# youtalk/opencv-ar

Hardware: AMD Instinct MI355X
Metric: frames/sec at 1920x1080, 16 markers/frame; 1/2/4/8 MI355X (higher is better)
Workload: dtype u8

## Files before the change

include/ocvar_hip.h:

```cpp
#ifndef OCVAR_HIP_H
#define OCVAR_HIP_H

#include <stddef.h>
#include <stdint.h>

#ifdef __cplusplus
extern "C" {
#endif

typedef struct { int width, height; double cameraMatrix[9]; double distCoeffs[5]; double glProjection[16]; } OcvarCamera;
typedef struct { int width, height; double scale; long long code[4]; } OcvarTemplate;
typedef struct {
    double glMatrix[16]; int templateId; int markerId; double score; float square[8]; double aspectRatio;
} OcvarMarker;

typedef struct {
    int markerId, templateId, orient, valid;
    long long bit;
    float square[8];
    float patPoint[8];
} OcvarCandidate;

typedef struct OcvarHip OcvarHip;

// ... 195 lines not shown
int ocvar_hip_debug_binary(OcvarHip* ctx, int frame, uint8_t* h_bin );
int ocvar_hip_debug_masks(OcvarHip* ctx, int frame, uint8_t* h_masks );
int ocvar_hip_debug_frame_quads(OcvarHip* ctx, int frame, int* quads , int* n_quads);
int ocvar_hip_debug_candidates(OcvarHip* ctx, int frame, OcvarCandidate* cands, int max_cands, int* n_cands);
typedef struct OcvarCropRoi {
    int index, frame, owner, x0, y0, w, h;
} OcvarCropRoi;
int ocvar_hip_debug_crop_rois(OcvarHip* ctx, OcvarCropRoi* rois, int max_rois, int* n_rois);
int ocvar_hip_debug_crop_plane(OcvarHip* ctx, int roi, int masks, uint8_t* h_plane );

typedef struct OcvarStart {
    int roi, x, y, is_hole;
} OcvarStart;
int ocvar_hip_debug_starts(OcvarHip* ctx, int crop_pass, OcvarStart* starts, int max_starts, int* n_starts);

int ocvar_hip_debug_calibrate(OcvarHip* ctx, size_t bytes);

int ocvar_hip_stage_ms(OcvarHip* ctx, float* ms, int n);
int ocvar_hip_stage_stamps(OcvarHip* ctx, void* ref_event, float* ms, int n);
int ocvar_hip_counters(OcvarHip* ctx, long long* out, int n);

#ifdef __cplusplus
}
#endif
#endif
```

opencv-ar_amd/__init__.py:

```python
import ctypes as C
import os

import numpy as np

_HERE = os.path.dirname(os.path.abspath(__file__))
LIB_DIR = os.path.join(_HERE, "lib")
HIP_LIB = os.environ.get("OCVAR_HIP_LIB") or os.path.join(LIB_DIR, "libocvar_hip.so")
SYNTH_LIB = os.path.join(LIB_DIR, "libocvar_synth.so")
HOST_LIB = os.path.join(LIB_DIR, "libopencv-ar.so.1.0.0")

MAX_TEMPLATES, MAX_TEMPLATE_SIZES, MAX_QUADS, MAX_MARKERS = 4096, 16, 256, 64
MAX_QUADS_EX, MAX_QUADS_DENSE, MAX_MARKERS_DENSE = 1792, 16384, 4096

HIP_SYMBOLS = [
    "ocvar_hip_create", "ocvar_hip_create_ex", "ocvar_hip_create_dense", "ocvar_hip_max_markers", "ocvar_hip_capacity_flags", "ocvar_hip_gate_create", "ocvar_hip_gate_create_lanes", "ocvar_hip_gate_lanes", "ocvar_hip_gate_destroy", "ocvar_hip_set_gate", "ocvar_hip_ready", "ocvar_hip_set_result_limit",
    "ocvar_hip_pipe_create", "ocvar_hip_pipe_destroy", "ocvar_hip_pipe_last_error", "ocvar_hip_pipe_set_templates", "ocvar_hip_pipe_set_camera",
    "ocvar_hip_pipe_detect_device", "ocvar_hip_pipe_track_device", "ocvar_hip_pipe_submit", "ocvar_hip_pipe_collect", "ocvar_hip_pipe_in_flight", "ocvar_hip_pipe_set_result_limit", "ocvar_hip_set_input_format", "ocvar_hip_pipe_set_input_format", "ocvar_hip_set_corner_refine", "ocvar_hip_pipe_set_corner_refine", "ocvar_hip_enqueue_tracked", "ocvar_hip_build_info", "ocvar_hip_set_tuning", "ocvar_hip_destroy", "ocvar_hip_last_error", "ocvar_hip_set_templates", "ocvar_hip_set_camera",
    "ocvar_hip_detect_device", "ocvar_hip_enqueue", "ocvar_hip_collect", "ocvar_hip_detect_host", "ocvar_hip_find_squares",
    "ocvar_hip_debug_gray", "ocvar_hip_debug_binary", "ocvar_hip_debug_masks", "ocvar_hip_debug_frame_quads", "ocvar_hip_debug_candidates",
    "ocvar_hip_debug_crop_rois", "ocvar_hip_debug_crop_plane", "ocvar_hip_debug_starts",
    "ocvar_hip_stage_ms", "ocvar_hip_stream", "ocvar_hip_stage_stamps", "ocvar_hip_counters", "ocvar_hip_results_to_device", "ocvar_hip_results_to_device_ex", "ocvar_hip_debug_calibrate",
    "ocvar_hip_set_board", "ocvar_hip_board_poses", "ocvar_hip_board_poses_to_device",
    "ocvar_hip_set_overlay", "ocvar_hip_render", "ocvar_hip_render_records",
    "ocvar_hip_annotate_default_style", "ocvar_hip_annotate", "ocvar_hip_annotate_records",
    "ocvar_hip_patches", "ocvar_hip_patches_records",
    "ocvar_hip_undistort", "ocvar_hip_undistort_records",
    "ocvar_hip_flow_records",
    "ocvar_hip_yuv_to_frames", "ocvar_hip_frames_to_yuv",
    "ocvar_hip_resize", "ocvar_hip_scale_records",
    "ocvar_hip_orient", "ocvar_hip_orient_records", "ocvar_hip_orient_camera",
    "ocvar_hip_warp", "ocvar_hip_warp_records", "ocvar_hip_board_plane_maps",
    "ocvar_hip_levels_default_params", "ocvar_hip_levels",
]
INPUT_FORMATS = {"bgr": 0, "rgb": 1, "bgra": 2, "rgba": 3, "gray": 4}
FORMAT_BPP = {0: 3, 1: 3, 2: 4, 3: 4, 4: 1}
# ... 314 lines not shown
        lib.ocvar_hip_set_templates.argtypes = [vp, vp, i]
        lib.ocvar_hip_set_camera.argtypes = [vp, vp]
        lib.ocvar_hip_detect_device.argtypes = [vp, vp, i, i, i, sz, i, i, vp, vp, vp, vp, i]
        lib.ocvar_hip_enqueue.argtypes = [vp, vp, i, i, i, sz, i, i, vp, vp, vp]
        lib.ocvar_hip_collect.argtypes = [vp, vp, vp, i]
        lib.ocvar_hip_detect_host.argtypes = [vp, vp, i, i, i, sz, i, i, vp, vp, vp, vp, i]
        lib.ocvar_hip_find_squares.argtypes = [vp, vp, i, i, i, vp, i, vp]
        lib.ocvar_hip_debug_gray.argtypes = [vp, i, vp]
        lib.ocvar_hip_debug_binary.argtypes = [vp, i, vp]
        lib.ocvar_hip_debug_masks.argtypes = [vp, i, vp]
        lib.ocvar_hip_debug_frame_quads.argtypes = [vp, i, vp, vp]
        lib.ocvar_hip_debug_candidates.argtypes = [vp, i, vp, i, vp]
        lib.ocvar_hip_debug_crop_rois.argtypes = [vp, vp, i, vp]
        lib.ocvar_hip_debug_crop_plane.argtypes = [vp, i, i, vp]
        lib.ocvar_hip_debug_starts.argtypes = [vp, i, vp, i, vp]
        lib.ocvar_hip_stage_ms.argtypes = [vp, vp, i]
        lib.ocvar_hip_counters.argtypes = [vp, vp, i]
        lib.ocvar_hip_stage_stamps.argtypes = [vp, vp, vp, i]
        lib.ocvar_hip_stream.argtypes = [vp]
        lib.ocvar_hip_stream.restype = vp
        lib.ocvar_hip_results_to_device.argtypes = [vp, vp, vp, vp]
        lib.ocvar_hip_results_to_device_ex.argtypes = [vp, vp, vp, i, vp]
        lib.ocvar_hip_debug_calibrate.argtypes = [vp, sz]
        lib.ocvar_hip_set_board.argtypes = [vp, vp, i]
        lib.ocvar_hip_board_poses.argtypes = [vp, vp, i]
        lib.ocvar_hip_board_poses_to_device.argtypes = [vp, vp, vp]
        lib.ocvar_hip_set_overlay.argtypes = [vp, i, vp, i, i, i]
        lib.ocvar_hip_render.argtypes = [vp, vp, i, i, i, sz, i, vp]
        lib.ocvar_hip_render_records.argtypes = [vp, vp, i, i, i, sz, i, i, vp, vp, i, vp]
        lib.ocvar_hip_annotate_default_style.argtypes = [vp]
# ... 589 lines not shown
        return out

    def debug_crop_binary(self, roi):
        return self._debug_crop_plane(roi, False)

    def debug_crop_masks(self, roi):
        return self._debug_crop_plane(roi, True)

    def debug_starts(self, crop_pass=False):
        n = C.c_int(0)
        self._check(self._lib.ocvar_hip_debug_starts(self._ctx, int(bool(crop_pass)), None, 0, C.byref(n)), "debug_starts")
        out = np.zeros(max(n.value, 1), START_DTYPE)
        self._check(self._lib.ocvar_hip_debug_starts(self._ctx, int(bool(crop_pass)), _ptr(out), n.value, C.byref(n)), "debug_starts")
        return out[:n.value]

    def stage_ms(self):
        ms = np.zeros(12, np.float32)
        k = self._lib.ocvar_hip_stage_ms(self._ctx, _ptr(ms), 12)
        return ms[:max(k, 0)]

    def stream_ptr(self):
        return self._lib.ocvar_hip_stream(self._ctx)

    def stage_stamps(self, ref_event):
        ms = np.zeros(13, np.float32)
        k = self._lib.ocvar_hip_stage_stamps(self._ctx, ref_event, _ptr(ms), 13)
        return ms[:max(k, 0)]

    def counters(self, n=10):
        out = np.zeros(n, np.int64)
# ... 3 lines not shown
```

opencv-ar_amd/csrc/api.hip:

```cpp
#include "context.h"
#include "plan_core.h"
#include <algorithm>
#include <cstdlib>
#include <cstring>
#include <new>

using namespace ocvar;

static_assert(sizeof(TemplateRec) == sizeof(OcvarTemplate) && sizeof(TemplateRec) == 48, "CvarTemplate layout");
static_assert(MAX_SIZE_CLASSES == OCVAR_MAX_TEMPLATE_SIZES, "size classes");
static_assert(sizeof(CameraRec) == sizeof(OcvarCamera) && sizeof(CameraRec) == 248, "CvarCamera layout");
static_assert(sizeof(MarkerRec) == sizeof(OcvarMarker) && sizeof(MarkerRec) == 184, "CvarMarker layout");
static_assert(sizeof(BoardEntry) == sizeof(OcvarBoardMarker) && sizeof(BoardEntry) == 72, "OcvarBoardMarker layout");
static_assert(sizeof(BoardPose) == sizeof(OcvarBoardPose) && sizeof(BoardPose) == 192, "OcvarBoardPose layout");

template <typename T>
static int dev_alloc(OcvarHip* c, T** p, size_t n) {
    void* q = nullptr;
    HIP_TRY(c, hipMalloc(&q, n * sizeof(T) + 256));
    c->allocs.push_back(q);
    *p = static_cast<T*>(q);
    return OCVAR_OK;
}

// ... 39 lines not shown
    if ((rc = dev_alloc(c, &w.crop_live, (size_t)w.cap_long))) return rc;
    if ((rc = dev_alloc(c, &w.long_frame, (size_t)w.cap_long))) return rc;
    if ((rc = dev_alloc(c, &w.long_crop, (size_t)w.cap_long))) return rc;
    if ((rc = dev_alloc(c, &w.quads_frame, B * max_quads))) return rc;
    if ((rc = dev_alloc(c, &w.n_quads_frame, B))) return rc;
    if ((rc = dev_alloc(c, &w.squares, B * max_quads * 8))) return rc;
    if ((rc = dev_alloc(c, &w.n_squares, B))) return rc;
    if ((rc = dev_alloc(c, &w.crop_of, B * max_quads))) return rc;
    if ((rc = dev_alloc(c, &w.rois_crop, (size_t)w.cap_crop_rois))) return rc;
    if ((rc = dev_alloc(c, &w.tiles_crop, (size_t)w.cap_crop_tiles))) return rc;
    if ((rc = dev_alloc(c, &w.quads_crop, (size_t)w.cap_crop_quads))) return rc;
    if ((rc = dev_alloc(c, &w.best_crop, (size_t)w.cap_crop_rois))) return rc;
    if ((rc = dev_alloc(c, &w.crop_min_rest, (size_t)w.cap_crop_rois))) return rc;
    if ((rc = dev_alloc(c, &w.ring_frame, B))) return rc;
    if ((rc = dev_alloc(c, &w.ring_crop, (size_t)w.cap_crop_rois))) return rc;
    if ((rc = dev_alloc(c, &w.sq_recs, B * max_quads))) return rc;
    if ((rc = dev_alloc(c, &w.prev, B * M))) return rc;
    if ((rc = dev_alloc(c, &w.n_prev, B))) return rc;
    if ((rc = dev_alloc(c, &w.reserve, B * M))) return rc;
    if ((rc = dev_alloc(c, &w.n_reserve, B))) return rc;
    if ((rc = dev_alloc(c, &w.markers, B * M))) return rc;
    if ((rc = dev_alloc(c, &w.pose_jobs, B * M))) return rc;
    if (dense) {
        const int nc = w.track_gw * w.track_gh;
        if ((rc = dev_alloc(c, &w.sorted_starts, B * max_quads))) return rc;
        if ((rc = dev_alloc(c, &w.sq_tmp, B * max_quads * 8))) return rc;
        if ((rc = dev_alloc(c, &w.trk_cells, B * (nc + 1)))) return rc;
        if ((rc = dev_alloc(c, &w.trk_fill, B * nc))) return rc;
        if ((rc = dev_alloc(c, &w.trk_items, B * 4 * max_quads))) return rc;
        if ((rc = dev_alloc(c, &w.trk_next, B * (max_quads + 1)))) return rc;
        if ((rc = dev_alloc(c, &w.surv, B * max_quads))) return rc;
        if ((rc = dev_alloc(c, &w.src, B * M))) return rc;
    }
    if ((rc = dev_alloc(c, &w.n_markers, B))) return rc;
    if ((rc = dev_alloc(c, &w.templates, (size_t)MAXT))) return rc;
    if ((rc = dev_alloc(c, &w.sizes, (size_t)MAX_SIZE_CLASSES))) return rc;
    if ((rc = dev_alloc(c, &w.lut, (size_t)4 * MAXT))) return rc;
    if ((rc = dev_alloc(c, &w.group_off, (size_t)MAXT + 1))) return rc;
    if ((rc = dev_alloc(c, &w.group_members, (size_t)MAXT))) return rc;
    if ((rc = dev_alloc(c, &w.camera, (size_t)1))) return rc;
    if ((rc = dev_alloc(c, &w.counters, (size_t)CNT_COUNT))) return rc;

    w.crop_pixels = reinterpret_cast<unsigned long long*>(w.counters + CNT_CROP_PIXELS);
    HIP_TRY(c, hipMemset(w.n_prev, 0, B * sizeof(int)));
    HIP_TRY(c, hipMemset(w.counters, 0, CNT_COUNT * sizeof(int)));
    HIP_TRY(c, c->h_markers.reserve(B * M * sizeof(MarkerRec)));
    HIP_TRY(c, c->h_counts.reserve(B * sizeof(int)));
    HIP_TRY(c, c->h_prev.reserve(B * M * sizeof(MarkerRec)));
    HIP_TRY(c, c->h_prev_counts.reserve(B * sizeof(int)));
    HIP_TRY(c, c->h_counters.reserve(CNT_COUNT * sizeof(int)));
    return OCVAR_OK;
}

extern "C" int ocvar_hip_create(OcvarHip** out, int device, int max_width, int max_height, int max_batch) {
    return ocvar_hip_create_ex(out, device, max_width, max_height, max_batch, OCVAR_MAX_QUADS);
}

extern "C" int ocvar_hip_create_ex(OcvarHip** out, int device, int max_width, int max_height, int max_batch, int max_quads) {
    if (max_quads < 1 || max_quads > OCVAR_MAX_QUADS_EX) return OCVAR_E_ARG;
    return create_impl(out, device, max_width, max_height, max_batch, max_quads, OCVAR_MAX_MARKERS, false);
// ... 157 lines not shown
        return OCVAR_E_ARG;
    }
    HIP_TRY(c, hipSetDevice(c->device));
    c->batch_board = false;
    c->crops_ran = false;
    plan_batch(&w, r.width, r.height, n_frames, c->gate != nullptr,
               PlanOverrides{tuned(c, OCVAR_TUNE_CROP_PHASES, "OCVAR_CROP_PHASES"), tuned(c, OCVAR_TUNE_MID_STEPS, "OCVAR_MID_STEPS"),
                             tuned(c, OCVAR_TUNE_MID_BLOCKS, "OCVAR_MID_BLOCKS"), tuned(c, OCVAR_TUNE_LONG_BLOCKS, "OCVAR_LONG_BLOCKS"),
                             tuned(c, OCVAR_TUNE_SHORT_BLOCKS, "OCVAR_SHORT_BLOCKS"), tuned(c, OCVAR_TUNE_MIN_UNITS, "OCVAR_MIN_UNITS")});
    if (after && after != s && hipStreamQuery(after) != hipSuccess) {
        (void)hipGetLastError();
        HIP_TRY(c, c->ordered.ensure(hipEventDisableTiming));
        HIP_TRY(c, hipEventRecord(c->ordered, after));
        HIP_TRY(c, hipStreamWaitEvent(s, c->ordered, 0));
    }
    HIP_TRY(c, hipMemsetAsync(w.counters, 0, CNT_COUNT * sizeof(int), s));
    HIP_TRY(c, hipMemsetAsync(w.n_quads_frame, 0, n_frames * sizeof(int), s));
    if (r.prev && r.prev_counts && r.prev_on_device) {
        HIP_TRY(c, hipMemcpyAsync(w.prev, r.prev, (size_t)n_frames * w.maxm * sizeof(MarkerRec), hipMemcpyDeviceToDevice, s));
        HIP_TRY(c, hipMemcpyAsync(w.n_prev, r.prev_counts, n_frames * sizeof(int), hipMemcpyDeviceToDevice, s));
    } else if (r.prev && r.prev_counts) {
        std::memcpy(c->h_prev, r.prev, (size_t)n_frames * w.maxm * sizeof(MarkerRec));
        std::memcpy(c->h_prev_counts, r.prev_counts, n_frames * sizeof(int));
        HIP_TRY(c, hipMemcpyAsync(w.prev, c->h_prev, (size_t)n_frames * w.maxm * sizeof(MarkerRec), hipMemcpyHostToDevice, s));
        HIP_TRY(c, hipMemcpyAsync(w.n_prev, c->h_prev_counts, n_frames * sizeof(int), hipMemcpyHostToDevice, s));
    } else {
        HIP_TRY(c, hipMemsetAsync(w.n_prev, 0, n_frames * sizeof(int), s));
    }
    const int hp_mask = (int)knob_or(tuned(c, OCVAR_TUNE_HP_MASK, "OCVAR_HP_MASK"), HP_MASK_DEFAULT) & 0x1ff;
    if (hp_mask && !c->hp_stream) {
        int lo = 0, hi = 0;
// ... 1105 lines not shown
```

opencv-ar_amd/csrc/binarise.hip:

```cpp
#include "kernels.h"
#include "starts_core.h"
#include <cstdlib>
#include <type_traits>

#ifndef OCVAR_WAVES_F
#define OCVAR_WAVES_F 5
#endif
#ifndef OCVAR_ROWS_AHEAD_F
#define OCVAR_ROWS_AHEAD_F 2
#endif
#ifndef OCVAR_ROWS_AHEAD_F4
#define OCVAR_ROWS_AHEAD_F4 1
#endif
#ifndef OCVAR_BIN_WG_WAVES
#define OCVAR_BIN_WG_WAVES 1
#endif
#ifndef OCVAR_ROWS_AHEAD_C
#define OCVAR_ROWS_AHEAD_C 1
#endif
#ifndef OCVAR_WAVES_C
#define OCVAR_WAVES_C 5
#endif

namespace ocvar {
// ... 50 lines not shown
    if constexpr (B == 1) asm("v_cmp_lt_i32_sdwa vcc, sext(%1), %2 src0_sel:WORD_1 src1_sel:BYTE_1\n\tv_cndmask_b32_e64 %0, 0, 1, vcc" : "=v"(nib) : "v"(S), "v"(w) : "vcc");
    if constexpr (B == 2) asm("v_cmp_lt_i32_sdwa vcc, sext(%1), %2 src0_sel:WORD_1 src1_sel:BYTE_2\n\tv_cndmask_b32_e64 %0, 0, 1, vcc" : "=v"(nib) : "v"(S), "v"(w) : "vcc");
    if constexpr (B == 3) asm("v_cmp_lt_i32_sdwa vcc, sext(%1), %2 src0_sel:WORD_1 src1_sel:BYTE_3\n\tv_cndmask_b32_e64 %0, 0, 1, vcc" : "=v"(nib) : "v"(S), "v"(w) : "vcc");
}

struct MarchOut {
    uint8_t* gray;
    long long gray_stride;
    uint8_t* nbr;
    int ns;
    int roi;
    StartCand* cands;
    int* n_cands;
    int cap_cands;
    int* err;
};

constexpr int SRC_CROP = 5;
constexpr int src_bpp(int src) { return src == OCVAR_FMT_BGR || src == OCVAR_FMT_RGB ? 3 : src == OCVAR_FMT_BGRA || src == OCVAR_FMT_RGBA ? 4 : 1; }

template <int SRC, bool EDGE>
__device__ void march_unit(const uint8_t* src, long long src_stride, int x_org , int sw, int sh, int strip, int Y0, int Y1, const MarchOut& o,
                           unsigned* stage, uint8_t* rowbuf ) {
    constexpr bool FRAME = SRC != SRC_CROP;
    constexpr int BPP = src_bpp(SRC);
    constexpr bool FOUR = BPP == 4;
    const int lane = threadIdx.x & 63;
    const int XS = strip * SV - 4 * HL;
    const int c0 = XS + 4 * lane;
    const int pw = sw >> 1, ph_ = sh >> 1;
// ... 41 lines not shown
            const unsigned e = stage[i];
            if (base + i < o.cap_cands) {
                StartCand sc;
                sc.roi = o.roi;
                sc.pos = (int)(e & 0x7fffffffu);
                sc.is_hole = (int)(e >> 31);
                o.cands[base + i] = sc;
            } else {
                atomicOr(o.err, ERR_CAND_OVERFLOW);
            }
        }
        __builtin_amdgcn_fence(__ATOMIC_ACQ_REL, "workgroup");
        staged = 0;
    };

    const int tile_s = strip * (SV / NBR_TILE_W) + (lane >> 2);
    const unsigned flush_src = (unsigned)(lane < 60 ? lane >> 2 : 14) * 4u;
    const unsigned flush_dst = lane < 60 && tile_s * NBR_TILE_W < o.ns ? (unsigned)tile_s * NBR_TILE_BYTES + (unsigned)(lane & 3) * 16u : OOB;
    auto flush_tiles = [&](int ty) {
        __builtin_amdgcn_fence(__ATOMIC_ACQ_REL, "workgroup");
        int fl = lane;
        asm volatile("" : "+v"(fl));
        const int ftx = fl >> 2, fq = fl & 3;
        const unsigned wbits = starts_word_bits(ftx);
        unsigned w[4];
        {
            typedef unsigned v4u __attribute__((ext_vector_type(4)));
            v4u d;
#pragma unroll
            for (int i = 0; i < 4; i++) {
                const int r = NBR_TILE_H * ty + 4 * (lane & 3) + i - 1;
                const unsigned* p = reinterpret_cast<const unsigned*>(rowbuf + (r & (RING_ROWS - 1)) * 64 + flush_src);
                const unsigned p0 = p[0], p1 = p[1];
                const unsigned ww = __builtin_amdgcn_perm(p1 | (p1 >> 4), p0 | (p0 >> 4), 0x06040200u);
                w[i] = (unsigned)r <= (unsigned)Y1 ? ww & wbits : 0u;
                d[i] = (w[i] >> 7) & 0x3ffffu;
            }
            const unsigned so = (unsigned)wave_uniform((int)nbr_tile_off(0u, (unsigned)ty, o.ns));
            __builtin_amdgcn_raw_buffer_store_b128(d, nbr_rs, (int)(flush_dst + so), 0, BUF_NT);
        }
        const int nrows = wave_uniform(Y1 - NBR_TILE_H * ty < NBR_TILE_H ? Y1 - NBR_TILE_H * ty : NBR_TILE_H);
        const int col0 = strip * SV + NBR_TILE_W * ftx;
        const unsigned own = fl < 60 ? (EDGE ? starts_own_bits(col0, sw) : STARTS_OWN_BITS) : 0u;
        unsigned long long any, hole;
        starts_of_lane(w, up1(w[3]), 4 * fq - 1, nrows, own, any, hole);
        const unsigned pos0 = (unsigned)((NBR_TILE_H * ty + 4 * fq - 1) * o.ns + col0);
#pragma nounroll
        for (;;) {
            const unsigned long long mask = __ballot(any != 0ull);
            const int n = wave_uniform(__popcll(mask));
            if (n == 0) break;
            if (staged + n > MARCH_STAGE) flush();
            if (any != 0ull) {
                const unsigned k = (unsigned)__builtin_ctzll(any);
                stage[staged + __popcll(mask & ((1ull << lane) - 1ull))] = (pos0 + (k >> 4) * (unsigned)o.ns + (k & 15u)) | ((unsigned)(hole >> k) << 31);
                any &= any - 1ull;
            }
            staged += n;
// ... 305 lines not shown
    if (unit >= per_frame * ws.n_frames) return;
    const int f = unit / per_frame, rem = unit % per_frame;
    const int chunk = rem / ws.frame_strips, strip = rem % ws.frame_strips;
    const int Y0 = chunk * ws.frame_chunk_rows;
    const int Y1 = Y0 + ws.frame_chunk_rows < ws.sh ? Y0 + ws.frame_chunk_rows : ws.sh;
    MarchOut o;
    o.gray = ws.gray + (size_t)f * gray_plane_bytes(ws.W, ws.H);
    o.gray_stride = gray_pitch(ws.W);
    o.nbr = ws.nbr_frame + (size_t)f * nbr_plane_bytes(ws.ns, ws.sh);
    o.ns = ws.ns;
    o.roi = f;
    o.cands = ws.cands_frame;
    o.n_cands = ws.counters + CNT_FRAME_CANDS;
    o.cap_cands = ws.cap_frame_cands;
    o.err = ws.counters + CNT_ERR;
    const int w4 = wave_uniform((int)(threadIdx.x >> 6));
    const bool edge = strip == 0 || ((ws.sw - 1 - (strip * MARCH_STRIP - 4 * MARCH_HALO_L)) >> 2) <= 63;
    if (edge) march_unit<FMT, true>(bgr + (size_t)f * frame_stride, row_stride, 0, ws.sw, ws.sh, strip, Y0, Y1, o, stage[w4], rowbuf[w4]);
    else march_unit<FMT, false>(bgr + (size_t)f * frame_stride, row_stride, 0, ws.sw, ws.sh, strip, Y0, Y1, o, stage[w4], rowbuf[w4]);
}

__device__ __forceinline__ uint8_t grey_at(const uint8_t* p, int fmt) {
    if (fmt == OCVAR_FMT_GRAY) return p[0];
    const bool rev = fmt == OCVAR_FMT_RGB || fmt == OCVAR_FMT_RGBA;
    return (uint8_t)grey_of(p[rev ? 2 : 0], p[1], p[rev ? 0 : 2]);
}

__global__ __launch_bounds__(256) void grey_edges_kernel(Workspace ws, const uint8_t* bgr, int row_stride, size_t frame_stride, int fmt) {
    const int f = blockIdx.y;
    const uint8_t* src = bgr + (size_t)f * frame_stride;
// ... 44 lines not shown
        const TileDesc td = ws.tiles_crop[u];
        const Roi r = ws.rois_crop[td.roi];
        const int pitch = gray_pitch(ws.W);
        const uint8_t* src = ws.gray + (size_t)r.frame * gray_plane_bytes(ws.W, ws.H) + (size_t)r.y0 * pitch;
        const int Y1 = td.y0 + MARCH_CROP_ROWS < r.sh ? td.y0 + MARCH_CROP_ROWS : r.sh;
        MarchOut o;
        o.gray = nullptr;
        o.gray_stride = 0;
        o.nbr = ws.nbr_crop + r.nbr_off;
        o.ns = r.ns;
        o.roi = td.roi;
        o.cands = ws.cands_crop;
        o.n_cands = ws.counters + CNT_CROP_CANDS;
        o.cap_cands = ws.cap_crop_cands;
        o.err = ws.counters + CNT_ERR;
        march_unit<SRC_CROP, true>(src, pitch, r.x0, r.sw, r.sh, td.x0, td.y0, Y1, o, stage[wave], rowbuf[wave]);
    }
}

int input_format_bpp(int format) { return format >= OCVAR_FMT_BGR && format <= OCVAR_FMT_GRAY ? src_bpp(format) : 0; }

void launch_binarise_frames(const Workspace& ws, const uint8_t* d_bgr, int row_stride, size_t frame_stride, int grey_in_place,
                            int format, hipStream_t stream) {
    const int units = ws.frame_strips * ws.frame_chunks * ws.n_frames;
    if (units <= 0) return;
    const dim3 grid((units + BW - 1) / BW), block(64 * BW);
    switch (format) {
    case OCVAR_FMT_RGB: hipLaunchKernelGGL(binarise_frames_kernel<OCVAR_FMT_RGB>, grid, block, 0, stream, ws, d_bgr, row_stride, frame_stride); break;
    case OCVAR_FMT_BGRA: hipLaunchKernelGGL(binarise_frames_kernel<OCVAR_FMT_BGRA>, grid, block, 0, stream, ws, d_bgr, row_stride, frame_stride); break;
    case OCVAR_FMT_RGBA: hipLaunchKernelGGL(binarise_frames_kernel<OCVAR_FMT_RGBA>, grid, block, 0, stream, ws, d_bgr, row_stride, frame_stride); break;
// ... 16 lines not shown
```

opencv-ar_amd/csrc/debug.hip:

```cpp
#include "context.h"
#include <cstring>

using namespace ocvar;

extern "C" int ocvar_hip_debug_gray(OcvarHip* c, int frame, uint8_t* h) {
    if (!c || !h || frame < 0 || frame >= c->ws.n_frames) return OCVAR_E_ARG;
    HIP_TRY(c, hipSetDevice(c->device));
    const int W = c->ws.W, H = c->ws.H, pitch = gray_pitch(W);
    const size_t plane = (size_t)gray_plane_bytes(W, H);
    std::vector<uint8_t> g(plane);
    HIP_TRY(c, hipMemcpy(g.data(), c->ws.gray + frame * plane, plane, hipMemcpyDeviceToHost));
    for (int y = 0; y < H; y++)
        for (int x = 0; x < W; x++) h[(size_t)y * W + x] = g[(size_t)y * pitch + gray_col(x)];
    return OCVAR_OK;
}

static int plane_to_host(OcvarHip* c, int frame, uint8_t* h, bool masks) {
    if (!c || !h || frame < 0 || frame >= c->ws.n_frames) return OCVAR_E_ARG;
    HIP_TRY(c, hipSetDevice(c->device));
    const int sw = c->ws.sw, sh = c->ws.sh, ns = c->ws.ns;
    const size_t bytes = (size_t)nbr_plane_bytes(ns, sh);
    std::vector<uint8_t> nbr(bytes);
    HIP_TRY(c, hipMemcpy(nbr.data(), c->ws.nbr_frame + (size_t)frame * bytes, bytes, hipMemcpyDeviceToHost));
    for (int y = 0; y < sh; y++)
// ... 79 lines not shown
    std::vector<Roi> rois((size_t)(crop_pass && n_rois > 0 ? n_rois : 1));
    if (crop_pass && n_rois > 0) HIP_TRY(c, hipMemcpy(rois.data(), c->ws.rois_crop, (size_t)n_rois * sizeof(Roi), hipMemcpyDeviceToHost));
    for (int i = 0; i < k; i++) {
        const StartCand& s = sc[i];
        const int ns = crop_pass ? (s.roi >= 0 && s.roi < n_rois ? rois[s.roi].ns : 0) : c->ws.ns;
        if (s.roi < 0 || s.roi >= n_rois || ns <= 0 || s.pos < 0) {
            c->err = "ocvar_hip_debug_starts: a record of the start list does not belong to the batch";
            return OCVAR_E_ARG;
        }
        starts[i].roi = s.roi;
        starts[i].x = s.pos % ns;
        starts[i].y = s.pos / ns;
        starts[i].is_hole = s.is_hole;
    }
    *n_starts = n;
    return OCVAR_OK;
}

extern "C" int ocvar_hip_debug_candidates(OcvarHip* c, int frame, OcvarCandidate* cands, int max_cands, int* n_cands) {
    if (!c || !cands || !n_cands || frame < 0 || frame >= c->ws.n_frames) return OCVAR_E_ARG;
    HIP_TRY(c, hipSetDevice(c->device));
    int nsq = 0;
    HIP_TRY(c, hipMemcpy(&nsq, c->ws.n_squares + frame, sizeof(int), hipMemcpyDeviceToHost));
    if (nsq > c->ws.maxq) nsq = c->ws.maxq;
    const Workspace& w = c->ws;
    const Library& L = c->lib;
    const size_t first = (size_t)frame * w.maxq;
    std::vector<SquareRec> recs(nsq > 0 ? nsq : 1);
    std::vector<long long> codes((size_t)(nsq > 0 ? nsq : 1) * w.n_sizes);
    std::vector<int> match((size_t)(nsq > 0 ? nsq : 1) * w.max_match);
// ... 54 lines not shown
```

opencv-ar_amd/csrc/follow.hip:

```cpp
#include "kernels.h"
#include "walk_core.h"

namespace ocvar {

__device__ __forceinline__ int ticket_lane() {
    int l = (int)(threadIdx.x & 63);
    asm volatile("" : "+v"(l));
    return l;
}
__device__ __forceinline__ int uni(int v) { return __builtin_amdgcn_readfirstlane(v); }
__device__ __forceinline__ unsigned uni(unsigned v) { return (unsigned)__builtin_amdgcn_readfirstlane((int)v); }
__device__ __forceinline__ unsigned long long uni(unsigned long long v) {
    return ((unsigned long long)uni((unsigned)(v >> 32)) << 32) | uni((unsigned)v);
}
__device__ __forceinline__ double uni(double v) { return __longlong_as_double((long long)uni((unsigned long long)__double_as_longlong(v))); }

#ifdef OCVAR_PROF
#define PROF_NOW() __builtin_readcyclecounter()
#define PROF_DECL() unsigned long long prof_acc[16] = {0, 0, 0, 0, 0, 0, 0, 0, 0, 0, 0, 0, 0, 0, 0, 0}
#define PROF_ADD(slot, v) do { prof_acc[slot] += (unsigned long long)(v); } while (0)
#define PROF_FLUSH(base) do { if ((threadIdx.x & 63) == 0) for (int i_ = 0; i_ < 16; i_++) if (i_ != 7) atomicAdd(reinterpret_cast<unsigned long long*>(ws.counters + CNT_PROF) + (base) + i_, prof_acc[i_]); } while (0)
#else
#define PROF_NOW() 0ull
#define PROF_DECL() do { } while (0)
// ... 462 lines not shown
        if (CROP && route == 1) atomicMin(ws.crop_min_rest + c.roi, c.pos);
        collect(0, o_n0, route == 1, c);
        collect(1, o_n1, route == 2, c);
        if (CROP) collect(2, o_n2, route == 3, c);
    }
    append(0, o_n0);
    append(1, o_n1);
    if (CROP) append(2, o_n2);
}

template <bool CROP>
__global__ __launch_bounds__(64) void ring_quads_kernel(Workspace ws) {
    int n = CROP ? ws.counters[CNT_CROP_ROIS] : ws.n_frames;
    if (CROP && n > ws.cap_crop_rois) n = ws.cap_crop_rois;
    int* ring = CROP ? ws.ring_crop : ws.ring_frame;
    const int lane = threadIdx.x;
    for (int roi = blockIdx.x; roi < n; roi += gridDim.x) {
        const PlaneRef pl = plane_of<CROP>(ws, roi);
        const int ns = uni(pl.ns), sh = uni(pl.sh), sw = uni(pl.img_w) & ~1;
        bool bad = sw < 8 || sh < 8;
        if (!bad) {
            const int tiles = ns >> 4;
            for (int i = lane; i < 2 * tiles; i += 64) {
                const int y = i < tiles ? 1 : sh - 2, xt = i < tiles ? i : i - tiles;
                const unsigned v = *reinterpret_cast<const unsigned*>(pl.nbr + nbr_win_off(xt << 4, y, ns) + 4);
                const int lo = (xt << 4) > 1 ? (xt << 4) : 1, hi = (xt << 4) + 15 < sw - 2 ? (xt << 4) + 15 : sw - 2;
                if (lo <= hi) {
                    const unsigned need = ((2u << (hi - lo)) - 1u) << (lo - (xt << 4) + 1);
                    if ((v & need) != need) bad = true;
                }
            }
            for (int y = 1 + lane; y <= sh - 2; y += 64)
                if (!nbr_bit(pl.nbr, 1, y, ns) || !nbr_bit(pl.nbr, sw - 2, y, ns)) bad = true;
        }
        const bool clean = __ballot(bad) == 0;
        if (lane == 0) {
            ring[roi] = clean ? 1 : 0;
            if (clean && (long long)(sw - 3) * (sh - 3) > 500) {
                const int pts[8] = {1, 1, 1, sh - 2, sw - 2, sh - 2, sw - 2, 1};
                const TraceStats st = stats_of_points(pts, 4);
                StartCand c;
                c.roi = roi;
                c.pos = ns + 1;
                c.is_hole = 0;
                DpSlice stack[DP_STACK];
                approximate_and_emit<CROP>(ws, c, pl, pts, 4, st.perimeter, stack);
            }
        }
    }
}

constexpr int MID_BLOCK = 32;
constexpr int POINT_ROW = MID_BLOCK + 1;
constexpr int FLUSH_W = MID_BLOCK <= 16 ? 16 : 32;
static_assert(FLUSH_W >= MID_BLOCK && 64 % FLUSH_W == 0, "a group of lanes covers a whole row of parked points");

template <bool CROP>
__global__ __launch_bounds__(FOLLOW_THREADS) void follow_mid_kernel(Workspace ws, int phase) {
    __shared__ WaveScratch scratch[FW];
    __shared__ unsigned parked[FW][64 * POINT_ROW];
    __shared__ unsigned step_tab[64];
    if (threadIdx.x < 64u) step_tab[threadIdx.x] = lean_table_entry(threadIdx.x);
// ... 446 lines not shown
                        wave_finish_packed<CROP, false>(ws, c, pl, reinterpret_cast<const unsigned*>(big), lt2.npts, staged[wave], &scratch[wave]);
                    } else if (lane == 0) {
                        atomicOr(ws.counters + CNT_ERR, ERR_TRACE_OVERRUN);
                    }
                }
            } else {
                __builtin_amdgcn_fence(__ATOMIC_ACQ_REL, "workgroup");
                if (lt.npts <= LDS_PTS) wave_finish_packed<CROP, true>(ws, c, pl, reinterpret_cast<const unsigned*>(slab), lt.npts, staged[wave], &scratch[wave]);
                else wave_finish_packed<CROP, false>(ws, c, pl, reinterpret_cast<const unsigned*>(slab), lt.npts, staged[wave], &scratch[wave]);
            }
        }
    }
}

void launch_ring_quads_frames(const Workspace& ws, hipStream_t stream) {
    hipLaunchKernelGGL(ring_quads_kernel<false>, dim3(ws.n_frames < 4096 ? ws.n_frames : 4096), dim3(64), 0, stream, ws);
}
void launch_ring_quads_crops(const Workspace& ws, hipStream_t stream) {
    hipLaunchKernelGGL(ring_quads_kernel<true>, dim3(ws.n_frames >= 128 ? 4096 : ws.n_frames * 32), dim3(64), 0, stream, ws);
}
void launch_follow_frames(const Workspace& ws, hipStream_t stream) {
    hipLaunchKernelGGL(follow_kernel<false>, dim3(ws.short_blocks * (4 / FW)), dim3(FOLLOW_THREADS), 0, stream, ws);
}
void launch_follow_crops(const Workspace& ws, hipStream_t stream) {
    hipLaunchKernelGGL(follow_kernel<true>, dim3(ws.short_blocks * (4 / FW)), dim3(FOLLOW_THREADS), 0, stream, ws);
}
void launch_follow_mid_frames(const Workspace& ws, hipStream_t stream) {
    hipLaunchKernelGGL(follow_mid_kernel<false>, dim3(ws.mid_blocks * (4 / FW)), dim3(FOLLOW_THREADS), 0, stream, ws, 0);
}
void launch_follow_mid_crops(const Workspace& ws, hipStream_t stream) {
    if (ws.crop_phases == 1) {
        hipLaunchKernelGGL(follow_mid_kernel<true>, dim3(ws.mid_blocks * (4 / FW)), dim3(FOLLOW_THREADS), 0, stream, ws, 0);
        return;
    }
// ... 16 lines not shown
```

opencv-ar_amd/csrc/kernels.h:

```cpp
#pragma once
#include "hd.h"
#include "decode_core.h"
#include "pose_core.h"
#include "tail_core.h"
#include "refine_core.h"
#include "board_core.h"
#include "overlay_core.h"
#include "annotate_core.h"
#include "patch_core.h"
#include "undistort_core.h"
#include "yuv_core.h"
#include "resize_core.h"
#include "orient_core.h"
#include "warp_core.h"
#include "levels_core.h"
#include "flow_core.h"
#include "croplist_core.h"
#include "ocvar_hip.h"

namespace ocvar {

constexpr int MAXQ_DEFAULT = OCVAR_MAX_QUADS;
constexpr int MAXM = OCVAR_MAX_MARKERS;
constexpr int MAXT = OCVAR_MAX_TEMPLATES;
// ... 23 lines not shown

struct SquareRec {
    float square[8];
    float patPoint[8];
    int n_match;
    int pad;
};

enum { CNT_FRAME_CANDS = 0, CNT_CROP_ROIS = 1, CNT_CROP_TILES = 2, CNT_CROP_CANDS = 3,
       CNT_POOL_INTS = 4 , CNT_CROP_QUADS = 6, CNT_TICKET_F = 7, CNT_TICKET_C = 8, CNT_ERR = 9,
       CNT_CROP_PIXELS = 10 , CNT_LONG_F = 12, CNT_LONG_C = 13, CNT_TICKET_LF = 14, CNT_TICKET_LC = 15,
       CNT_MID_F = 16, CNT_MID_C = 17, CNT_TICKET_MF = 18, CNT_TICKET_MC = 19, CNT_TICKET_BC = 20, CNT_MID_C_FIRST = 21, CNT_TICKET_MC2 = 22,
       CNT_POSE_JOBS = 23,
       CNT_PROF = 24 ,
       CNT_CROP_EARLY = 88, CNT_CROP_REST = 89, CNT_CROP_LIVE = 90 , CNT_COUNT = 92 };

struct Workspace {
    int max_w, max_h, max_batch;
    int maxq;
    int maxm;
    int dense;
    int track_gw, track_gh;
    int decode_slices;
    int order_chunk;
    int cap_frame_cands, cap_crop_cands, cap_crop_rois, cap_crop_tiles, cap_crop_quads;
    long long cap_pool_ints, cap_crop_pixels;
    int W, H, sw, sh, ns, n_frames, n_templates;
    int n_sizes, n_groups, max_match;
    int crop_phases;
    int crop_steps_cap;
// ... 18 lines not shown
    int* pool;
    int* slab;
    int* slab3;
    QuadRec* quads_frame;
    int* n_quads_frame;
    float* squares;
    int* n_squares;
    int* crop_of;
    Roi* rois_crop;
    TileDesc* tiles_crop;
    unsigned long long* crop_pixels;
    QuadRec* quads_crop;
    unsigned long long* best_crop;
    int* ring_frame;
    int* ring_crop;
    int* crop_min_rest;
    SquareRec* sq_recs;
    long long* sq_codes;
    int* sq_match;
    MarkerRec* prev;
    int* n_prev;
    int* reserve;
    int* n_reserve;
    int* pose_jobs;
    MarkerRec* markers;
    int* sorted_starts;
    float* sq_tmp;
    int* trk_cells;
    int* trk_fill;
    int* trk_items;
// ... 164 lines not shown
```

opencv-ar_amd/csrc/order.hip:

```cpp
#include "kernels.h"

namespace ocvar {

__device__ __forceinline__ void setup_crop(const Workspace& ws, int f, int i, const float* sq) {
    int quad[8];
    for (int k = 0; k < 8; k++) quad[k] = (int)sq[k];
    int x0, y0, cw, ch, roi_index = -1;
    crop_rect(quad, ws.W, ws.H, &x0, &y0, &cw, &ch);
    const int sw = cw & ~1, sh = ch & ~1, ns = (sw + 15) & ~15;
    if (sw >= 2 && sh >= 2) {
        const int r = atomicAdd(ws.counters + CNT_CROP_ROIS, 1);
        const long long plane = nbr_plane_bytes(ns, sh);
        const long long off = (long long)atomicAdd(ws.crop_pixels, (unsigned long long)plane);
        const int ntx = (sw + MARCH_STRIP - 1) / MARCH_STRIP, nty = (sh + MARCH_CROP_ROWS - 1) / MARCH_CROP_ROWS;
        if (r >= ws.cap_crop_rois || off + plane > ws.cap_crop_pixels) {
            atomicOr(ws.counters + CNT_ERR, ERR_CROP_OVERFLOW);
        } else {
            const int tbase = atomicAdd(ws.counters + CNT_CROP_TILES, ntx * nty);
            if (tbase + ntx * nty > ws.cap_crop_tiles) {
                atomicOr(ws.counters + CNT_ERR, ERR_TILE_OVERFLOW);
            } else {
                Roi roi;
                roi.frame = f; roi.x0 = x0; roi.y0 = y0; roi.w = cw; roi.h = ch; roi.sw = sw; roi.sh = sh; roi.ns = ns;
                roi.owner = i; roi.nbr_off = off;
                ws.rois_crop[r] = roi;
                ws.best_crop[r] = ~0ull;
                ws.crop_min_rest[r] = 0x7fffffff;
                ws.ring_crop[r] = 0;
                for (int t = 0; t < ntx * nty; t++) {
                    TileDesc td;
                    td.roi = r; td.x0 = t % ntx; td.y0 = (t / ntx) * MARCH_CROP_ROWS;
                    ws.tiles_crop[tbase + t] = td;
                }
                roi_index = r;
            }
        }
    }
    ws.crop_of[(size_t)f * ws.maxq + i] = roi_index;
}

__global__ __launch_bounds__(256) void order_and_crops_kernel(Workspace ws) {
    extern __shared__ int order_lds[];
    int* s_start = order_lds;
// ... 183 lines not shown
```

opencv-ar_amd/csrc/starts_core.h:

```cpp
#pragma once
#include "hd.h"

namespace ocvar {

OCVAR_HD unsigned starts_outer(unsigned c, unsigned a) { return c & ~(c << 1) & ~((a << 1) | a | (a >> 1)) & ~((c >> 1) & (a >> 2)); }
OCVAR_HD unsigned starts_hole(unsigned c, unsigned a) { return (c << 1) & ~c & a & ((c >> 1) | (a >> 1)); }

constexpr int STARTS_WORD_LEAD = 8;
constexpr unsigned STARTS_OWN_BITS = 0x00ffff00u;
constexpr int STARTS_STRIP_TILES = 15;

OCVAR_HD unsigned starts_word_bits(int tile_in_strip) { return tile_in_strip == STARTS_STRIP_TILES - 1 ? ~(1u << 25) : ~0u; }

OCVAR_HD unsigned starts_own_bits(int col0, int sw) {
    const int n = sw - col0;
    return n <= 0 ? 0u : n >= NBR_TILE_W ? STARTS_OWN_BITS : ((1u << n) - 1u) << STARTS_WORD_LEAD;
}

OCVAR_HD void starts_of_lane(const unsigned w[4], unsigned above, int qrow, int nrows, unsigned own, unsigned long long& any, unsigned long long& hole) {
    unsigned m[4], h[4];
    unsigned a = above;
    for (int i = 0; i < 4; i++) {
        const unsigned c = w[i];
        const unsigned sel = (unsigned)(qrow + i) < (unsigned)nrows ? own : 0u;
        h[i] = starts_hole(c, a) & sel;
        m[i] = (starts_outer(c, a) & sel) | h[i];
        a = c;
    }
    const unsigned m01 = (m[0] >> STARTS_WORD_LEAD) | (m[1] << (16 - STARTS_WORD_LEAD)), m23 = (m[2] >> STARTS_WORD_LEAD) | (m[3] << (16 - STARTS_WORD_LEAD));
    const unsigned h01 = (h[0] >> STARTS_WORD_LEAD) | (h[1] << (16 - STARTS_WORD_LEAD)), h23 = (h[2] >> STARTS_WORD_LEAD) | (h[3] << (16 - STARTS_WORD_LEAD));
    any = (unsigned long long)m01 | ((unsigned long long)m23 << 32);
    hole = (unsigned long long)h01 | ((unsigned long long)h23 << 32);
}

}
```

Before: 264,000.

## Detect open image border rings during marching instead of rescanning in ring kernel

The binarise/march kernel now checks, while it already holds each tile's words, whether the one-pixel border ring of a frame or crop is broken, and records a per-ROI ring_open flag. The ring_quads kernel then reads that flag with one thread per ROI instead of a full wave rescanning the top, bottom and side border pixels of each plane. Launch grids for ring_quads shrink to match. This adds ballot and predicate work inside the hot march loop for edge and border tile rows, plus extra counter-block memset and allocation, and a debug accessor.

```diff
diff --git a/include/ocvar_hip.h b/include/ocvar_hip.h
--- a/include/ocvar_hip.h
+++ b/include/ocvar_hip.h
@@ -233,6 +233,8 @@
 } OcvarStart;
 int ocvar_hip_debug_starts(OcvarHip* ctx, int crop_pass, OcvarStart* starts, int max_starts, int* n_starts);
 
+int ocvar_hip_debug_rings(OcvarHip* ctx, int crop_pass, int* ring_open, int* ring, int max_rois, int* n_rois);
+
 int ocvar_hip_debug_calibrate(OcvarHip* ctx, size_t bytes);
 
 int ocvar_hip_stage_ms(OcvarHip* ctx, float* ms, int n);
diff --git a/opencv-ar_amd/__init__.py b/opencv-ar_amd/__init__.py
--- a/opencv-ar_amd/__init__.py
+++ b/opencv-ar_amd/__init__.py
@@ -18,7 +18,7 @@
     "ocvar_hip_pipe_detect_device", "ocvar_hip_pipe_track_device", "ocvar_hip_pipe_submit", "ocvar_hip_pipe_collect", "ocvar_hip_pipe_in_flight", "ocvar_hip_pipe_set_result_limit", "ocvar_hip_set_input_format", "ocvar_hip_pipe_set_input_format", "ocvar_hip_set_corner_refine", "ocvar_hip_pipe_set_corner_refine", "ocvar_hip_enqueue_tracked", "ocvar_hip_build_info", "ocvar_hip_set_tuning", "ocvar_hip_destroy", "ocvar_hip_last_error", "ocvar_hip_set_templates", "ocvar_hip_set_camera",
     "ocvar_hip_detect_device", "ocvar_hip_enqueue", "ocvar_hip_collect", "ocvar_hip_detect_host", "ocvar_hip_find_squares",
     "ocvar_hip_debug_gray", "ocvar_hip_debug_binary", "ocvar_hip_debug_masks", "ocvar_hip_debug_frame_quads", "ocvar_hip_debug_candidates",
-    "ocvar_hip_debug_crop_rois", "ocvar_hip_debug_crop_plane", "ocvar_hip_debug_starts",
+    "ocvar_hip_debug_crop_rois", "ocvar_hip_debug_crop_plane", "ocvar_hip_debug_starts", "ocvar_hip_debug_rings",
     "ocvar_hip_stage_ms", "ocvar_hip_stream", "ocvar_hip_stage_stamps", "ocvar_hip_counters", "ocvar_hip_results_to_device", "ocvar_hip_results_to_device_ex", "ocvar_hip_debug_calibrate",
     "ocvar_hip_set_board", "ocvar_hip_board_poses", "ocvar_hip_board_poses_to_device",
     "ocvar_hip_set_overlay", "ocvar_hip_render", "ocvar_hip_render_records",
@@ -363,6 +363,7 @@
         lib.ocvar_hip_debug_crop_rois.argtypes = [vp, vp, i, vp]
         lib.ocvar_hip_debug_crop_plane.argtypes = [vp, i, i, vp]
         lib.ocvar_hip_debug_starts.argtypes = [vp, i, vp, i, vp]
+        lib.ocvar_hip_debug_rings.argtypes = [vp, i, vp, vp, i, vp]
         lib.ocvar_hip_stage_ms.argtypes = [vp, vp, i]
         lib.ocvar_hip_counters.argtypes = [vp, vp, i]
         lib.ocvar_hip_stage_stamps.argtypes = [vp, vp, vp, i]
@@ -982,6 +983,13 @@
         self._check(self._lib.ocvar_hip_debug_starts(self._ctx, int(bool(crop_pass)), _ptr(out), n.value, C.byref(n)), "debug_starts")
         return out[:n.value]
 
+    def debug_rings(self, crop_pass=False):
+        n = C.c_int(0)
+        self._check(self._lib.ocvar_hip_debug_rings(self._ctx, int(bool(crop_pass)), None, None, 0, C.byref(n)), "debug_rings")
+        ring_open, ring = np.zeros(max(n.value, 1), np.int32), np.zeros(max(n.value, 1), np.int32)
+        self._check(self._lib.ocvar_hip_debug_rings(self._ctx, int(bool(crop_pass)), _ptr(ring_open), _ptr(ring), n.value, C.byref(n)), "debug_rings")
+        return ring_open[:n.value], ring[:n.value]
+
     def stage_ms(self):
         ms = np.zeros(12, np.float32)
         k = self._lib.ocvar_hip_stage_ms(self._ctx, _ptr(ms), 12)
diff --git a/opencv-ar_amd/csrc/api.hip b/opencv-ar_amd/csrc/api.hip
--- a/opencv-ar_amd/csrc/api.hip
+++ b/opencv-ar_amd/csrc/api.hip
@@ -77,6 +77,7 @@
     if ((rc = dev_alloc(c, &w.crop_min_rest, (size_t)w.cap_crop_rois))) return rc;
     if ((rc = dev_alloc(c, &w.ring_frame, B))) return rc;
     if ((rc = dev_alloc(c, &w.ring_crop, (size_t)w.cap_crop_rois))) return rc;
+    if ((rc = dev_alloc(c, &w.ring_open_crop, (size_t)w.cap_crop_rois))) return rc;
     if ((rc = dev_alloc(c, &w.sq_recs, B * max_quads))) return rc;
     if ((rc = dev_alloc(c, &w.prev, B * M))) return rc;
     if ((rc = dev_alloc(c, &w.n_prev, B))) return rc;
@@ -102,11 +103,12 @@
     if ((rc = dev_alloc(c, &w.group_off, (size_t)MAXT + 1))) return rc;
     if ((rc = dev_alloc(c, &w.group_members, (size_t)MAXT))) return rc;
     if ((rc = dev_alloc(c, &w.camera, (size_t)1))) return rc;
-    if ((rc = dev_alloc(c, &w.counters, (size_t)CNT_COUNT))) return rc;
+    if ((rc = dev_alloc(c, &w.counters, counters_block_ints(max_batch)))) return rc;
+    w.ring_open_frame = w.counters + CNT_RING_OPEN;
 
     w.crop_pixels = reinterpret_cast<unsigned long long*>(w.counters + CNT_CROP_PIXELS);
     HIP_TRY(c, hipMemset(w.n_prev, 0, B * sizeof(int)));
-    HIP_TRY(c, hipMemset(w.counters, 0, CNT_COUNT * sizeof(int)));
+    HIP_TRY(c, hipMemset(w.counters, 0, counters_block_ints(max_batch) * sizeof(int)));
     HIP_TRY(c, c->h_markers.reserve(B * M * sizeof(MarkerRec)));
     HIP_TRY(c, c->h_counts.reserve(B * sizeof(int)));
     HIP_TRY(c, c->h_prev.reserve(B * M * sizeof(MarkerRec)));
@@ -294,7 +296,7 @@
         HIP_TRY(c, hipEventRecord(c->ordered, after));
         HIP_TRY(c, hipStreamWaitEvent(s, c->ordered, 0));
     }
-    HIP_TRY(c, hipMemsetAsync(w.counters, 0, CNT_COUNT * sizeof(int), s));
+    HIP_TRY(c, hipMemsetAsync(w.counters, 0, counters_block_ints(n_frames) * sizeof(int), s));
     HIP_TRY(c, hipMemsetAsync(w.n_quads_frame, 0, n_frames * sizeof(int), s));
     if (r.prev && r.prev_counts && r.prev_on_device) {
         HIP_TRY(c, hipMemcpyAsync(w.prev, r.prev, (size_t)n_frames * w.maxm * sizeof(MarkerRec), hipMemcpyDeviceToDevice, s));
diff --git a/opencv-ar_amd/csrc/binarise.hip b/opencv-ar_amd/csrc/binarise.hip
--- a/opencv-ar_amd/csrc/binarise.hip
+++ b/opencv-ar_amd/csrc/binarise.hip
@@ -88,6 +88,7 @@
     int* n_cands;
     int cap_cands;
     int* err;
+    int* ring_open;
 };
 
 constexpr int SRC_CROP = 5;
@@ -159,9 +160,11 @@
         staged = 0;
     };
 
-    const int tile_s = strip * (SV / NBR_TILE_W) + (lane >> 2);
-    const unsigned flush_src = (unsigned)(lane < 60 ? lane >> 2 : 14) * 4u;
-    const unsigned flush_dst = lane < 60 && tile_s * NBR_TILE_W < o.ns ? (unsigned)tile_s * NBR_TILE_BYTES + (unsigned)(lane & 3) * 16u : OOB;
+    int ul = lane;
+    asm volatile("" : "+v"(ul));
+    const int tile_s = strip * (SV / NBR_TILE_W) + (ul >> 2);
+    const unsigned flush_src = (unsigned)(ul < 60 ? ul >> 2 : 14) * 4u;
+    const unsigned flush_dst = ul < 60 && tile_s * NBR_TILE_W < o.ns ? (unsigned)tile_s * NBR_TILE_BYTES + (unsigned)(ul & 3) * 16u : OOB;
     auto flush_tiles = [&](int ty) {
         __builtin_amdgcn_fence(__ATOMIC_ACQ_REL, "workgroup");
         int fl = lane;
@@ -187,6 +190,15 @@
         const int nrows = wave_uniform(Y1 - NBR_TILE_H * ty < NBR_TILE_H ? Y1 - NBR_TILE_H * ty : NBR_TILE_H);
         const int col0 = strip * SV + NBR_TILE_W * ftx;
         const unsigned own = fl < 60 ? (EDGE ? starts_own_bits(col0, sw) : STARTS_OWN_BITS) : 0u;
+        if (EDGE || ty == 0 || (unsigned)(sh - 2 - NBR_TILE_H * ty) < (unsigned)NBR_TILE_H) {
+            const unsigned rowb = fl < 60 ? ring_row_bits(col0, sw) : 0u, colb = ring_col_bits(ftx, strip * SV, sw);
+            const bool gap = ring_missing(w, 4 * fq - 1, nrows, NBR_TILE_H * ty, sh, rowb, colb) != 0u;
+            if (__ballot(gap) != 0ull) {
+                int slot = o.roi;
+                asm volatile("" : "+v"(slot));
+                if (fl == 0) o.ring_open[slot] = 1;
+            }
+        }
         unsigned long long any, hole;
         starts_of_lane(w, up1(w[3]), 4 * fq - 1, nrows, own, any, hole);
         const unsigned pos0 = (unsigned)((NBR_TILE_H * ty + 4 * fq - 1) * o.ns + col0);
@@ -522,6 +534,7 @@
     o.n_cands = ws.counters + CNT_FRAME_CANDS;
     o.cap_cands = ws.cap_frame_cands;
     o.err = ws.counters + CNT_ERR;
+    o.ring_open = ws.ring_open_frame;
     const int w4 = wave_uniform((int)(threadIdx.x >> 6));
     const bool edge = strip == 0 || ((ws.sw - 1 - (strip * MARCH_STRIP - 4 * MARCH_HALO_L)) >> 2) <= 63;
     if (edge) march_unit<FMT, true>(bgr + (size_t)f * frame_stride, row_stride, 0, ws.sw, ws.sh, strip, Y0, Y1, o, stage[w4], rowbuf[w4]);
@@ -596,6 +609,7 @@
         o.n_cands = ws.counters + CNT_CROP_CANDS;
         o.cap_cands = ws.cap_crop_cands;
         o.err = ws.counters + CNT_ERR;
+        o.ring_open = ws.ring_open_crop;
         march_unit<SRC_CROP, true>(src, pitch, r.x0, r.sw, r.sh, td.x0, td.y0, Y1, o, stage[wave], rowbuf[wave]);
     }
 }
diff --git a/opencv-ar_amd/csrc/debug.hip b/opencv-ar_amd/csrc/debug.hip
--- a/opencv-ar_amd/csrc/debug.hip
+++ b/opencv-ar_amd/csrc/debug.hip
@@ -117,6 +117,19 @@
         starts[i].is_hole = s.is_hole;
     }
     *n_starts = n;
+    return OCVAR_OK;
+}
+
+extern "C" int ocvar_hip_debug_rings(OcvarHip* c, int crop_pass, int* ring_open, int* ring, int max_rois, int* n_rois) {
+    if (!c || c->pending || !n_rois || max_rois < 0 || c->ws.n_frames < 1 || !c->h_counters.p) return OCVAR_E_ARG;
+    const int n = crop_pass ? crop_count(c) : c->ws.n_frames;
+    if (n < 0) return OCVAR_E_ARG;
+    HIP_TRY(c, hipSetDevice(c->device));
+    const size_t k = (size_t)(n < max_rois ? n : max_rois);
+    if (k > 0 && ring_open)
+        HIP_TRY(c, hipMemcpy(ring_open, crop_pass ? c->ws.ring_open_crop : c->ws.ring_open_frame, k * sizeof(int), hipMemcpyDeviceToHost));
+    if (k > 0 && ring) HIP_TRY(c, hipMemcpy(ring, crop_pass ? c->ws.ring_crop : c->ws.ring_frame, k * sizeof(int), hipMemcpyDeviceToHost));
+    *n_rois = n;
     return OCVAR_OK;
 }
 
diff --git a/opencv-ar_amd/csrc/follow.hip b/opencv-ar_amd/csrc/follow.hip
--- a/opencv-ar_amd/csrc/follow.hip
+++ b/opencv-ar_amd/csrc/follow.hip
@@ -500,38 +500,21 @@
     int n = CROP ? ws.counters[CNT_CROP_ROIS] : ws.n_frames;
     if (CROP && n > ws.cap_crop_rois) n = ws.cap_crop_rois;
     int* ring = CROP ? ws.ring_crop : ws.ring_frame;
-    const int lane = threadIdx.x;
-    for (int roi = blockIdx.x; roi < n; roi += gridDim.x) {
+    const int* ring_open = CROP ? ws.ring_open_crop : ws.ring_open_frame;
+    for (int roi = blockIdx.x * 64 + threadIdx.x; roi < n; roi += gridDim.x * 64) {
         const PlaneRef pl = plane_of<CROP>(ws, roi);
-        const int ns = uni(pl.ns), sh = uni(pl.sh), sw = uni(pl.img_w) & ~1;
-        bool bad = sw < 8 || sh < 8;
-        if (!bad) {
-            const int tiles = ns >> 4;
-            for (int i = lane; i < 2 * tiles; i += 64) {
-                const int y = i < tiles ? 1 : sh - 2, xt = i < tiles ? i : i - tiles;
-                const unsigned v = *reinterpret_cast<const unsigned*>(pl.nbr + nbr_win_off(xt << 4, y, ns) + 4);
-                const int lo = (xt << 4) > 1 ? (xt << 4) : 1, hi = (xt << 4) + 15 < sw - 2 ? (xt << 4) + 15 : sw - 2;
-                if (lo <= hi) {
-                    const unsigned need = ((2u << (hi - lo)) - 1u) << (lo - (xt << 4) + 1);
-                    if ((v & need) != need) bad = true;
-                }
-            }
-            for (int y = 1 + lane; y <= sh - 2; y += 64)
-                if (!nbr_bit(pl.nbr, 1, y, ns) || !nbr_bit(pl.nbr, sw - 2, y, ns)) bad = true;
-        }
-        const bool clean = __ballot(bad) == 0;
-        if (lane == 0) {
-            ring[roi] = clean ? 1 : 0;
-            if (clean && (long long)(sw - 3) * (sh - 3) > 500) {
-                const int pts[8] = {1, 1, 1, sh - 2, sw - 2, sh - 2, sw - 2, 1};
-                const TraceStats st = stats_of_points(pts, 4);
-                StartCand c;
-                c.roi = roi;
-                c.pos = ns + 1;
-                c.is_hole = 0;
-                DpSlice stack[DP_STACK];
-                approximate_and_emit<CROP>(ws, c, pl, pts, 4, st.perimeter, stack);
-            }
+        const int sh = pl.sh, sw = pl.img_w & ~1;
+        const bool clean = sw >= 8 && sh >= 8 && ring_open[roi] == 0;
+        ring[roi] = clean ? 1 : 0;
+        if (clean && (long long)(sw - 3) * (sh - 3) > 500) {
+            const int pts[8] = {1, 1, 1, sh - 2, sw - 2, sh - 2, sw - 2, 1};
+            const TraceStats st = stats_of_points(pts, 4);
+            StartCand c;
+            c.roi = roi;
+            c.pos = pl.ns + 1;
+            c.is_hole = 0;
+            DpSlice stack[DP_STACK];
+            approximate_and_emit<CROP>(ws, c, pl, pts, 4, st.perimeter, stack);
         }
     }
 }
@@ -1008,10 +991,10 @@
 }
 
 void launch_ring_quads_frames(const Workspace& ws, hipStream_t stream) {
-    hipLaunchKernelGGL(ring_quads_kernel<false>, dim3(ws.n_frames < 4096 ? ws.n_frames : 4096), dim3(64), 0, stream, ws);
+    hipLaunchKernelGGL(ring_quads_kernel<false>, dim3((ws.n_frames + 63) / 64), dim3(64), 0, stream, ws);
 }
 void launch_ring_quads_crops(const Workspace& ws, hipStream_t stream) {
-    hipLaunchKernelGGL(ring_quads_kernel<true>, dim3(ws.n_frames >= 128 ? 4096 : ws.n_frames * 32), dim3(64), 0, stream, ws);
+    hipLaunchKernelGGL(ring_quads_kernel<true>, dim3(ws.n_frames >= 512 ? 256 : (ws.n_frames + 1) / 2), dim3(64), 0, stream, ws);
 }
 void launch_follow_frames(const Workspace& ws, hipStream_t stream) {
     hipLaunchKernelGGL(follow_kernel<false>, dim3(ws.short_blocks * (4 / FW)), dim3(FOLLOW_THREADS), 0, stream, ws);
diff --git a/opencv-ar_amd/csrc/kernels.h b/opencv-ar_amd/csrc/kernels.h
--- a/opencv-ar_amd/csrc/kernels.h
+++ b/opencv-ar_amd/csrc/kernels.h
@@ -61,6 +61,8 @@
        CNT_POSE_JOBS = 23,
        CNT_PROF = 24 ,
        CNT_CROP_EARLY = 88, CNT_CROP_REST = 89, CNT_CROP_LIVE = 90 , CNT_COUNT = 92 };
+constexpr int CNT_RING_OPEN = 128;
+constexpr size_t counters_block_ints(int n_frames) { return (size_t)CNT_RING_OPEN + (((size_t)n_frames + 3) & ~(size_t)3); }
 
 struct Workspace {
     int max_w, max_h, max_batch;
@@ -109,6 +111,8 @@
     unsigned long long* best_crop;
     int* ring_frame;
     int* ring_crop;
+    int* ring_open_frame;
+    int* ring_open_crop;
     int* crop_min_rest;
     SquareRec* sq_recs;
     long long* sq_codes;
diff --git a/opencv-ar_amd/csrc/order.hip b/opencv-ar_amd/csrc/order.hip
--- a/opencv-ar_amd/csrc/order.hip
+++ b/opencv-ar_amd/csrc/order.hip
@@ -27,6 +27,7 @@
                 ws.best_crop[r] = ~0ull;
                 ws.crop_min_rest[r] = 0x7fffffff;
                 ws.ring_crop[r] = 0;
+                ws.ring_open_crop[r] = 0;
                 for (int t = 0; t < ntx * nty; t++) {
                     TileDesc td;
                     td.roi = r; td.x0 = t % ntx; td.y0 = (t / ntx) * MARCH_CROP_ROWS;
diff --git a/opencv-ar_amd/csrc/starts_core.h b/opencv-ar_amd/csrc/starts_core.h
--- a/opencv-ar_amd/csrc/starts_core.h
+++ b/opencv-ar_amd/csrc/starts_core.h
@@ -33,4 +33,27 @@
     hole = (unsigned long long)h01 | ((unsigned long long)h23 << 32);
 }
 
+OCVAR_HD unsigned ring_row_bits(int col0, int sw) {
+    const int lo = col0 > 1 ? col0 : 1, hi = col0 + NBR_TILE_W - 1 < sw - 2 ? col0 + NBR_TILE_W - 1 : sw - 2;
+    return lo <= hi ? ((2u << (hi - lo)) - 1u) << (lo - col0 + STARTS_WORD_LEAD) : 0u;
 }
+OCVAR_HD unsigned ring_col_bits(int tx, int strip0, int sw) {
+    const int last = sw - 2 - strip0;
+    const int tx_last = (unsigned)last < (unsigned)(STARTS_STRIP_TILES * NBR_TILE_W) ? last / NBR_TILE_W : -1;
+    const unsigned first_bit = strip0 == 0 ? 2u << STARTS_WORD_LEAD : 0u, last_bit = 1u << ((last & (NBR_TILE_W - 1)) + STARTS_WORD_LEAD);
+    return (tx == 0 ? first_bit : 0u) | (tx == tx_last ? last_bit : 0u);
+}
+OCVAR_HD bool ring_tile_row_between(int row0, int sh) { return row0 - 1 >= 1 && row0 + NBR_TILE_H <= sh - 2; }
+OCVAR_HD unsigned ring_missing(const unsigned w[4], int qrow, int nrows, int row0, int sh, unsigned rowb, unsigned colb) {
+    if (ring_tile_row_between(row0, sh)) return colb & ~(w[0] & w[1] & w[2] & w[3]);
+    const int j1 = 1 - row0, j2 = sh - 2 - row0;
+    unsigned miss = 0u;
+    for (int i = 0; i < 4; i++) {
+        const int j = qrow + i;
+        const unsigned need = j == j1 || j == j2 ? rowb : j > j1 && j < j2 ? colb : 0u;
+        if ((unsigned)j < (unsigned)nrows) miss |= need & ~w[i];
+    }
+    return miss;
+}
+
+}
```

Result: no change. 264,600, median of 4 (+0.2%).
